# BAMresearch/fenics-constitutive

Hardware: AMD Instinct MI355X
Metric: quadrature-point stress updates/sec (Mpts/s) + % HBM roofline, 1/2/4/8 GPU (higher is better)
Workload: dtype f64; 1 GPU; von_mises_mixed: von_mises_3d FULL-3D, 100000000 pts/GPU device-resident, committed->trial evaluate, packed sparse history; points_per_gpu=100000000, points_total=100000000, parallelism=shard1

## Files before the change

fenics-constitutive_amd/_build.py:

```python

from __future__ import annotations

import os
import shutil
import subprocess
import sys

HERE = os.path.dirname(os.path.abspath(__file__))
CSRC = os.path.join(HERE, "csrc")
LIBDIR = os.path.join(HERE, "lib")
LIB = os.path.join(LIBDIR, "libfcamd.so")
SOURCES = ["fcamd_kernels.hip", "fcamd_aux_kernels.hip", "fcamd_capi.cpp", "fcamd_hostpath.cpp", "fcamd_hosttangent.cpp", "fcamd_multigpu.cpp", "fcamd_memory.cpp", "fcamd_multi.cpp"]
KERNEL_HEADERS = [os.path.join("kernels", h) for h in (
    "tile_io.h", "tangent_writers.h", "wrapped_io.h", "history_rows.h", "law_linear_elasticity.h", "law_sls.h",
    "law_von_mises.h", "law_comfe_mises.h", "law_drucker_prager.h", "law_lowdim.h", "stress_wrapped.h", "param_source.h")]
HEADERS = ["fcamd_internal.h", "fcamd_host.h", os.path.join("..", "..", "include", "fcamd.h"), os.path.join("..", "..", "include", "fcamd_multi.h"), *KERNEL_HEADERS]
ARCH = "gfx950"
FLAGS = ["-O3", "-std=c++17", "-fPIC", "-shared", "-pthread", "-ffp-contract=off", "-Wall", "-Wno-unused-function"]


HASHFILE = os.path.join(LIBDIR, "libfcamd.srchash")


def _source_hash() -> str:
    import hashlib

    h = hashlib.sha256(" ".join([ARCH, *FLAGS]).encode())
    for f in SOURCES + HEADERS:
        with open(os.path.join(CSRC, f), "rb") as fh:
            h.update(fh.read())
    return h.hexdigest()


KERNEL_SOURCES = ["fcamd_kernels.hip", "fcamd_internal.h", *KERNEL_HEADERS]
KERNEL_FLAGS = [f for f in FLAGS if f not in ("-pthread", "-fPIC", "-shared", "-Wall", "-Wno-unused-function")]
KERNEL_HASHFILE = os.path.join(LIBDIR, "libfcamd.kernelhash")


def _code_only(text: str) -> str:
    import re

    text = re.sub(r"/\*.*?\*/", " ", text, flags=re.S)
    text = re.sub(r"//[^\n]*", " ", text)
    return " ".join(text.split())


def kernel_hash(read=None) -> str:
    import hashlib

    if read is None:
        def read(f):
            with open(os.path.join(CSRC, f)) as fh:
                return fh.read()

    h = hashlib.sha256(" ".join([ARCH, *KERNEL_FLAGS]).encode())
    for f in KERNEL_SOURCES:
        h.update(f.encode() + b"\0" + _code_only(read(f)).encode() + b"\0")
    return h.hexdigest()


def built_kernel_hash():
    try:
        with open(KERNEL_HASHFILE) as fh:
            return fh.read().strip()
    except OSError:
        return None


def _stale() -> bool:
    if not (os.path.exists(LIB) and os.path.exists(HASHFILE)):
        return True
    with open(HASHFILE) as fh:
        return fh.read().strip() != _source_hash()


def build_library(force: bool = False, verbose: bool = False, keep_temps: bool = False) -> str:
    if not force and not _stale():
        return LIB
    hipcc = shutil.which("hipcc") or "/opt/rocm/bin/hipcc"
    if not os.path.exists(hipcc):
        raise RuntimeError("hipcc not found; cannot build libfcamd.so")
    os.makedirs(LIBDIR, exist_ok=True)
    tmp = f"{LIB}.{os.getpid()}.tmp"
    cmd = [hipcc, f"--offload-arch={ARCH}", *FLAGS]
    if keep_temps:
        bdir = os.path.join(CSRC, "build")
        os.makedirs(bdir, exist_ok=True)
        cmd += [f"-save-temps={'obj'}", "-Rpass-analysis=kernel-resource-usage"]
        tmp = os.path.join(bdir, "libfcamd.so")
    cmd += ["-o", tmp, *[os.path.join(CSRC, s) for s in SOURCES]]
    if verbose:
        print(" ".join(cmd), file=sys.stderr)
    r = subprocess.run(cmd, capture_output=True, text=True)
    if r.returncode != 0:
        raise RuntimeError(f"hipcc failed ({r.returncode}):\n{r.stdout}\n{r.stderr}")
    if keep_temps:
        shutil.copyfile(tmp, LIB + ".cp")
        os.replace(LIB + ".cp", LIB)
        sys.stderr.write(r.stderr)
# ... 14 lines not shown
```

fenics-constitutive_amd/csrc/fcamd_capi.cpp:

```cpp
#include <algorithm>
#include <chrono>
#include <cmath>
#include <cstdarg>
#include <cstdio>
#include <cstdlib>
#include <cstring>
#include <new>
#include <string>

#include "fcamd_host.h"

using namespace fcamd;

namespace fcamd {

thread_local std::string g_last_error;

int fail(int status, const char* fmt, ...) {
    char buf[512];
    va_list ap;
    va_start(ap, fmt);
    vsnprintf(buf, sizeof(buf), fmt, ap);
    va_end(ap);
    g_last_error = buf;
    return status;
}

}

namespace {

constexpr int kMaskedRowMaxVonMises = 20;
constexpr int kMaskedRowMaxRows7 = 16;

static_assert(fcamd::kCounterSlots == FCAMD_COUNTER_SLOTS, "public and internal counter layout differ");

constexpr double kFactorPy = 0x1.6a09e667f3bccp-1;
constexpr double kFactorRs = 0x1.6a09e667f3bcdp-1;

bool law_info(int id, LawInfo* li) {
    switch (id) {
        case FCAMD_LINEAR_ELASTICITY: *li = {2, 0, {}, false}; return true;
        case FCAMD_VON_MISES_3D: *li = {5, 2, {{"eps_n", 6}, {"alpha", 1}}, false}; return true;
        case FCAMD_SPRING_MAXWELL: *li = {4, 2, {{"strain_visco", 6}, {"strain", 6}}, true}; return true;
        case FCAMD_SPRING_KELVIN: *li = {4, 2, {{"strain_visco", 6}, {"strain", 6}}, true}; return true;
        case FCAMD_COMFE_LINEAR_ELASTICITY: *li = {2, 0, {}, false}; return true;
        case FCAMD_COMFE_MISES_PLASTICITY: *li = {4, 1, {{"history", 7}}, false}; return true;
        case FCAMD_COMFE_DRUCKER_PRAGER: *li = {5, 1, {{"history", 7}}, false}; return true;
        case FCAMD_COMFE_DRUCKER_PRAGER_HYPERBOLIC: *li = {6, 1, {{"history", 7}}, false}; return true;
        default: return false;
    }
}


void lame(double E, double nu, double* mu, double* lam) {
    *mu = E / (2.0 * (1.0 + nu));
    *lam = E * nu / ((1.0 + nu) * (1.0 - 2.0 * nu));
}

void elastic_tangent_full(double E, double nu, double D[36]) {
    double mu, lam;
    lame(E, nu, &mu, &lam);
    for (int i = 0; i < 36; ++i) D[i] = 0.0;
    for (int i = 0; i < 3; ++i)
        for (int j = 0; j < 3; ++j) D[6 * i + j] = (i == j) ? 2.0 * mu + lam : lam;
    for (int i = 3; i < 6; ++i) D[6 * i + i] = 2.0 * mu;
}

Dims dims_of(int constraint) {
    switch (constraint) {
        case FCAMD_UNIAXIAL_STRAIN:
        case FCAMD_UNIAXIAL_STRESS: return {1, 1, 1};
        case FCAMD_PLANE_STRAIN:
        case FCAMD_PLANE_STRESS: return {4, 4, 2};
        default: return {9, 6, 3};
    }
}

void elastic_tangent(double E, double nu, int constraint, double D[36]) {
    for (int i = 0; i < 36; ++i) D[i] = 0.0;
    double mu, lam;
    lame(E, nu, &mu, &lam);
    switch (constraint) {
        case FCAMD_FULL: elastic_tangent_full(E, nu, D); break;
        case FCAMD_PLANE_STRAIN:
            for (int i = 0; i < 3; ++i)
                for (int j = 0; j < 3; ++j) D[4 * i + j] = (i == j) ? 2.0 * mu + lam : lam;
            D[15] = 2.0 * mu;
            break;
        case FCAMD_PLANE_STRESS: {
            const double c = E / (1 - std::pow(nu, 2.0));
            const double M[16] = {1.0, nu, 0.0, 0.0, nu, 1.0, 0.0, 0.0, 0.0, 0.0, 0.0, 0.0, 0.0, 0.0, 0.0, (1.0 - nu)};
            for (int i = 0; i < 16; ++i) D[i] = c * M[i];
// ... 96 lines not shown
            sc.s[5] = mu0 / (tau * mu1);
            sc.s[6] = lam0 / (tau * 2 * mu1);
            const double w0 = 1 - mu0 / (tau * mu1 * factor);
            for (int i = 0; i < 36; ++i) {
                tb.a[i] = D0[i];
                tb.c[i] = w0 * D0[i];
            }
            break;
        }
        case FCAMD_COMFE_LINEAR_ELASTICITY: {
            const double mu = p[0], kappa = p[1];
            double soo[36], pvol[36], pdev[36];
            comfe_projections(soo, pvol, pdev);
            sc.s[0] = kFactorRs;
            for (int i = 0; i < 36; ++i) tb.a[i] = (2.0 * mu) * pdev[i] + (3.0 * kappa) * pvol[i];
            for (int i = 0; i < 6; ++i)
                for (int j = 0; j < 6; ++j) tb.c[6 * j + i] = tb.a[6 * i + j];
            break;
        }
        case FCAMD_COMFE_MISES_PLASTICITY: {
            const double mu = p[0], kappa = p[1], y_0 = p[2], h = p[3];
            double soo[36], pvol[36], pdev[36];
            comfe_projections(soo, pvol, pdev);
            sc.s[0] = kFactorRs;
            sc.s[1] = mu;
            sc.s[2] = kappa;
            sc.s[3] = y_0;
            sc.s[4] = h;
            sc.s[5] = 2. * mu;
            sc.s[6] = 3. * mu + h;
            sc.s[7] = std::sqrt(3. / 2.);
            sc.s[8] = 3. * mu;
            sc.s[9] = 1.0 / (1.0 + (h / (3.0 * mu)));
            for (int i = 0; i < 36; ++i) {
                tb.a[i] = kappa * soo[i];
                tb.b[i] = pdev[i];
            }
            break;
        }
        case FCAMD_COMFE_DRUCKER_PRAGER:
        case FCAMD_COMFE_DRUCKER_PRAGER_HYPERBOLIC: {
            const bool hyper = m->law == FCAMD_COMFE_DRUCKER_PRAGER_HYPERBOLIC;
            const double mu = p[0], kappa = p[1], a_ = p[2], b = p[3];
            const double d = hyper ? p[4] : 0.0, b_flow = hyper ? p[5] : p[4];
            double soo[36], pvol[36], pdev[36];
            comfe_projections(soo, pvol, pdev);
            sc.s[0] = kFactorRs;
            sc.s[1] = mu;
            sc.s[2] = kappa;
            sc.s[3] = a_;
            sc.s[4] = b;
            sc.s[5] = b_flow;
            sc.s[6] = d * d;
            sc.s[7] = 2.0 * mu;
            sc.s[8] = std::sqrt(2.0 / 3.0);
            sc.s[9] = 1.0 / (4.0 * mu);
            sc.s[10] = 1.0 / (9.0 * kappa);
            for (int i = 0; i < 36; ++i) {
                tb.a[i] = soo[i];
                tb.b[i] = pdev[i];
                tb.c[i] = (2.0 * mu) * pdev[i] + (3.0 * kappa) * pvol[i];
            }
            break;
        }
    }
}

void options_from_env(Options* o) {
    auto geti = [](const char* name, long long dflt) {
        const char* e = getenv(name);
        return (e && *e) ? atoll(e) : dflt;
    };
    o->masked_max = (int)geti("FCAMD_MASKED_MAX", -1);
    o->batch_kernel = geti("FCAMD_BATCH_KERNEL", 1) != 0;
    o->host_chunk = geti("FCAMD_HOST_CHUNK", 0);
    o->host_slots = (int)std::min<long long>(fcamd_context::kSlots, std::max<long long>(1, geti("FCAMD_HOST_SLOTS", fcamd_context::kSlots)));
    o->zero_copy = geti("FCAMD_ZERO_COPY", 1) != 0;
    o->zero_copy_grad = geti("FCAMD_ZERO_COPY_GRAD", 1) != 0;
    o->bounce_max = std::max<long long>(0, geti("FCAMD_BOUNCE_MAX", 256 << 10));
    o->host_tangent_threads = (int)geti("FCAMD_HOST_TANGENT_THREADS", -1);
    o->host_tangent_min_points = std::max<long long>(0, geti("FCAMD_HOST_TANGENT_MIN", 1 << 16));
    o->host_tangent_chunk = std::max<long long>(0, geti("FCAMD_HOST_TANGENT_CHUNK", 0));
    o->host_tangent_streams = (int)std::max<long long>(1, std::min<long long>(fcamd_context::kSlots, geti("FCAMD_HOST_TANGENT_STREAMS", 1)));
}

void constants_for(fcamd_model* m, double del_t) {
    if (m->const_valid && (m->const_del_t == del_t || !m->info.needs_del_t)) return;
    fill_constants(m, del_t, m->sc, m->tb);
    m->const_del_t = del_t;
    m->const_valid = true;
}

bool law_counts(int law) { return law == FCAMD_VON_MISES_3D || law >= FCAMD_COMFE_MISES_PLASTICITY; }

int timing_begin(fcamd_model* m) {
    fcamd_context* c = m->ctx;
    m->timed = c->timing;
    m->host_ms = -1.0f;
    if (m->timed) {
        if (law_counts(m->law)) HIP_TRY(hipMemsetAsync(m->d_counters, 0, kCounterBytes, c->stream));
        HIP_TRY(hipEventRecord(m->ev0, c->stream));
    }
    return FCAMD_OK;
}
int timing_end(fcamd_model* m) {
    if (m->timed) HIP_TRY(hipEventRecord(m->ev1, m->ctx->stream));
    return FCAMD_OK;
}

}

namespace fcamd {
static bool is_split(const fcamd_model* m, int flags) { return (flags & FCAMD_EVAL_SPLIT_HISTORY) != 0 && has_split_history(m->law); }

int validate_call(const fcamd_model* m, double del_t, int64_t n, const void* grad,
                  const void* stress_prev, const void* stress, const void* const* hist_prev,
                  const void* const* hist, int n_hist, int flags) {
    if (!m) return fail(FCAMD_ERR_BAD_ARG, "model handle is NULL");
    if (n < 0) return fail(FCAMD_ERR_SIZE, "negative number of quadrature points");
    if ((flags & FCAMD_EVAL_SPLIT_HISTORY) && !has_split_history(m->law))
        return fail(FCAMD_ERR_UNSUPPORTED, "FCAMD_EVAL_SPLIT_HISTORY exists for the laws with one [scalar, eps_p(6)] history row per point");
    if (n_hist < 0 || n_hist > FCAMD_MAX_HISTORY)
        return fail(FCAMD_ERR_SIZE, "n_hist = %d: 0 .. %d history fields exist", n_hist, FCAMD_MAX_HISTORY);
    if (m->info.n_hist == 0 && n_hist != 0)
        return fail(FCAMD_ERR_SIZE, "law has no history, got %d history fields", n_hist);
    if (m->info.n_hist > 0) {
        const int expected = (flags & FCAMD_EVAL_SPLIT_HISTORY) ? 2 : m->info.n_hist;
        if (!hist || !hist_prev || n_hist == 0)
            return fail(FCAMD_ERR_NULL_HISTORY, "history must not be None");
        if (n_hist != expected)
            return fail(FCAMD_ERR_SIZE, "law expects %d history fields, got %d", expected,
                        n_hist);
        for (int k = 0; k < n_hist; ++k)
            if (n > 0 && (!hist[k] || !hist_prev[k]))
                return fail(FCAMD_ERR_NULL_HISTORY, "history must not be None");
    }
    if (m->info.needs_del_t && !(del_t > 0.0))
        return fail(FCAMD_ERR_DEL_T, "Time step must be defined and positive.");
    if (n > 0 && (!grad || !stress || !stress_prev))
        return fail(FCAMD_ERR_BAD_ARG, "grad_del_u / stress pointer is NULL");
    return FCAMD_OK;
}

int check_protocol(const fcamd_model* m, int64_t n, const fcamd_eval_args* x) {
    if (x->flags & ~(FCAMD_EVAL_SPARSE_TANGENT | FCAMD_EVAL_SPLIT_HISTORY | FCAMD_EVAL_PACKED_HISTORY | FCAMD_EVAL_PARAM_FIELDS |
                     FCAMD_EVAL_GRAD_ON_DEVICE))
        return fail(FCAMD_ERR_UNSUPPORTED, "unknown FCAMD_EVAL_* flag in 0x%x (2, FCAMD_EVAL_DELTA_HISTORY of ABI 0.3, was removed in 0.4)", x->flags);
    if (x->history_mask && !has_sparse_history(m->law))
        return fail(FCAMD_ERR_UNSUPPORTED, "sparse trial history exists for the plasticity laws only");
    if ((x->flags & FCAMD_EVAL_PACKED_HISTORY) && n > 0) {
        const bool split = is_split(m, x->flags);
        if (m->law != FCAMD_VON_MISES_3D && !split)
            return fail(FCAMD_ERR_UNSUPPORTED, "FCAMD_EVAL_PACKED_HISTORY exists for VonMises3D and, with FCAMD_EVAL_SPLIT_HISTORY, for the "
                                               "comfe-rs plasticity laws");
        if (!x->history_mask || !x->packed_mask_prev || !x->packed_mask)
            return fail(FCAMD_ERR_BAD_ARG, "FCAMD_EVAL_PACKED_HISTORY needs history_mask, packed_mask_prev and packed_mask");
        if (x->parent_rows && m->law != FCAMD_VON_MISES_3D)
            return fail(FCAMD_ERR_UNSUPPORTED, "FCAMD_EVAL_PACKED_HISTORY with parent_rows: VonMises3D only");
        const int kd = split ? 1 : 0;
        if (x->history[kd] == x->history_prev[kd] || x->packed_mask == x->packed_mask_prev)
            return fail(FCAMD_ERR_BAD_ARG, "FCAMD_EVAL_PACKED_HISTORY needs trial plastic-strain and mask arrays of their own");
    }
    if (!aligned16(x->stress) || !aligned16(x->stress_prev))
        return fail(FCAMD_ERR_ALIGN, "device arrays must be 16-byte aligned");
    for (int k = 0; k < x->n_hist; ++k)
        if (!aligned16(x->history[k]) || !aligned16(x->history_prev[k]))
// ... 77 lines not shown

static bool host_mapped(fcamd_context* c, const void* p) {
    const char* q = static_cast<const char*>(p);
    if (c->bounce_dev && q >= c->bounce_dev && q < c->bounce_dev + c->bounce_bytes) return true;
    std::lock_guard<std::recursive_mutex> lock(c->host_mu);
    for (const auto& kv : c->registered)
        if (kv.second.dev && q >= kv.second.dev && q < kv.second.dev + kv.second.bytes) return true;
    return false;
}

static void fill_args(fcamd_model* m, double del_t, int64_t n, const Launch& l, EvalArgs& a) {
    a.grad = l.grad;
    a.stress_in = l.stress_prev;
    a.stress_out = l.stress;
    a.stress_out2 = l.stress2;
    a.tangent = l.tangent;
    const bool split = is_split(m, l.flags);
    const int nh = split ? 2 : m->info.n_hist;
    a.h0_in = nh > 0 ? l.hist_prev[0] : nullptr;
    a.h0_out = nh > 0 ? l.hist[0] : nullptr;
    a.h1_in = nh > 1 ? l.hist_prev[1] : nullptr;
    a.h1_out = nh > 1 ? l.hist[1] : nullptr;
    a.rows = l.rows;
    a.cache3d = nullptr;
    a.hmask = l.hmask;
    a.flags = split ? FCAMD_EVAL_SPLIT_HISTORY : 0;
    if (l.hmask) {
        if (l.tangent) a.flags |= l.flags & FCAMD_EVAL_SPARSE_TANGENT;
        if ((a.flags & FCAMD_EVAL_SPARSE_TANGENT) && host_mapped(m->ctx, l.tangent)) a.flags |= kFlagExactTangentRows;
        if ((m->law == FCAMD_VON_MISES_3D || (split && !l.rows)) && l.emask_prev && l.emask) a.flags |= l.flags & FCAMD_EVAL_PACKED_HISTORY;
    }
    if (m->ctx->twin_masks && m->law == FCAMD_VON_MISES_3D && !l.rows && (a.flags & FCAMD_EVAL_PACKED_HISTORY)) {
        a.flags |= 64;
        a.cache3d = reinterpret_cast<double*>(m->ctx->twin_masks);
    }
    if (l.tangent && (l.flags & kFlagTangentParamsHost)) a.flags = (a.flags & ~FCAMD_EVAL_SPARSE_TANGENT) | kFlagTangentParamsHost;
    a.emask_in = l.emask_prev;
    a.emask_out = l.emask;
    a.n = n;
    a.counters = l.counters ? l.counters : m->d_counters;
    const Options& o = m->ctx->opt;
    a.masked_max = o.masked_max >= 0 ? o.masked_max
                                     : ((m->law == FCAMD_VON_MISES_3D || split) ? kMaskedRowMaxVonMises : kMaskedRowMaxRows7);
    constants_for(m, del_t);
    a.sc = m->sc;
    a.tb = m->tb;
}

const double* const* fields_of(const fcamd_eval_args* x) {
    return (x->flags & FCAMD_EVAL_PARAM_FIELDS) ? reinterpret_cast<const double* const*>(x->stress_3d) : nullptr;
}

bool has_fields(const fcamd_model* m, const double* const* fields) {
    if (!fields) return false;
    for (int k = 0; k < m->info.n_params; ++k)
        if (fields[k]) return true;
    return false;
}

int check_fields(const fcamd_model* m, const double* const* fields) {
    if (!has_fields(m, fields)) return FCAMD_OK;
    if (!law_has_field_kernels(m->law) || m->constraint != FCAMD_FULL)
        return fail(FCAMD_ERR_UNSUPPORTED, "per-point parameter fields exist for LinearElasticityModel (FULL), LinearElasticity3D, VonMises3D "
                                           "and MisesPlasticityLinearHardening3D (model %d, constraint %d)", m->law, m->constraint);
    for (int k = 0; k < m->info.n_params; ++k)
        if (!aligned16(fields[k])) return fail(FCAMD_ERR_ALIGN, "parameter field %d must be 16-byte aligned", k);
    return FCAMD_OK;
}

static void field_args_for(const fcamd_model* m, const double* const* fields, int64_t p0, FieldArgs& f) {
    std::memset(&f, 0, sizeof(f));
    for (int k = 0; k < m->info.n_params; ++k) {
        f.f[k] = fields[k] ? fields[k] + p0 : nullptr;
        f.v[k] = m->params[k];
    }
}

static void field_tables(const fcamd_model* m, EvalArgs& a) {
    if (m->law != FCAMD_VON_MISES_3D && m->law != FCAMD_COMFE_MISES_PLASTICITY) return;
    for (int i = 0; i < 6; ++i)
        for (int j = 0; j < 6; ++j) a.tb.a[6 * i + j] = (i < 3 && j < 3) ? 1.0 : 0.0;
}

int enqueue(fcamd_model* m, double del_t, int64_t n, const Launch& l, hipStream_t stream, bool reset_counters) {
    EvalArgs a;
    fill_args(m, del_t, n, l, a);
    const bool per_point = has_fields(m, l.fields);
    if (per_point) {
        a.flags &= ~64;
        a.cache3d = nullptr;
        field_tables(m, a);
    }
    if ((reset_counters || l.counters) && law_counts(m->law)) HIP_TRY(hipMemsetAsync(a.counters, 0, kCounterBytes, stream));
    if (n == 0) return FCAMD_OK;
    const int grid = grid_for(m, n);
    (void)hipGetLastError();
    if (per_point) {
        FieldArgs f;
        field_args_for(m, l.fields, l.field_p0, f);
        HIP_TRY(launch_evaluate_fields(m->law, a, f, grid, stream));
        return FCAMD_OK;
    }
    HIP_TRY(launch_evaluate(m->law, m->dims.gdim, a, grid, stream));
    return FCAMD_OK;
}
}

namespace fcamd {
void constants_for_call(fcamd_model* m, double del_t) { constants_for(m, del_t); }

void sum_counters(const fcamd_model* m, fcamd_stats* out) {
    out->n_nonconverged = out->n_plastic = out->n_newton_iters = out->n_domain = 0;
    out->kernel_ms = -1.0;
    for (int s = 0; s < fcamd::kCounterSlots; ++s) {
        out->n_nonconverged += m->h_counters[4 * s + 0];
        out->n_plastic += m->h_counters[4 * s + 1];
        out->n_newton_iters += m->h_counters[4 * s + 2];
        out->n_domain += m->h_counters[4 * s + 3];
    }
}

int enqueue_counters_download(fcamd_model* m, hipStream_t stream) {
    HIP_TRY(hipMemcpyAsync(m->h_counters, m->d_counters, kCounterBytes, hipMemcpyDeviceToHost, stream));
    return FCAMD_OK;
}

int read_stats(fcamd_model* m, hipStream_t stream, fcamd_stats* out) {
    int st = enqueue_counters_download(m, stream);
    if (st != FCAMD_OK) return st;
    HIP_TRY(hipStreamSynchronize(stream));
    if (out) sum_counters(m, out);
    return FCAMD_OK;
}
}

static int evaluate_wrapped(fcamd_model* m, int wrapper_constraint, double del_t, int64_t n, const double* grad_lo, double* stress_lo,
                            double* tangent_lo, double* stress_3d, double* const* hist, int n_hist);

extern "C" {

int fcamd_version(void) { return FCAMD_VERSION_MAJOR * 1000 + FCAMD_VERSION_MINOR; }

int fcamd_device_count(int* count) {
    if (!count) return fail(FCAMD_ERR_BAD_ARG, "NULL argument");
    *count = 0;
    if (hipGetDeviceCount(count) != hipSuccess) {
        (void)hipGetLastError();
        *count = 0;
    }
    return FCAMD_OK;
}

const char* fcamd_last_error(void) { return g_last_error.c_str(); }

int fcamd_context_create(int device, void* stream, fcamd_context** out) {
    if (!out) return fail(FCAMD_ERR_BAD_ARG, "out is NULL");
    *out = nullptr;
    int count = 0;
    HIP_TRY(hipGetDeviceCount(&count));
    if (device < 0 || device >= count)
        return fail(FCAMD_ERR_BAD_ARG, "device %d out of range (%d devices)", device, count);
    HIP_TRY(hipSetDevice(device));
    fcamd_context* c = new (std::nothrow) fcamd_context();
    if (!c) return fail(FCAMD_ERR_BAD_ARG, "out of host memory");
    c->device = device;
    options_from_env(&c->opt);
    const int st = [&]() -> int {
        hipDeviceProp_t prop;
        HIP_TRY(hipGetDeviceProperties(&prop, device));
        c->num_cu = prop.multiProcessorCount > 0 ? prop.multiProcessorCount : 256;
        if (stream) {
            c->stream = static_cast<hipStream_t>(stream);
        } else {
            HIP_TRY(hipStreamCreateWithFlags(&c->stream, hipStreamNonBlocking));
            c->owns_stream = true;
        }
        return FCAMD_OK;
    }();
    if (st != FCAMD_OK) {
        delete c;
        return st;
    }
    *out = c;
    return FCAMD_OK;
}

static int context_trim(fcamd_context* c) {
    if (!c) return fail(FCAMD_ERR_BAD_ARG, "context is NULL");
    std::lock_guard<std::recursive_mutex> lock(c->host_mu);
    HIP_TRY(hipSetDevice(c->device));
    for (int i = 0; i < fcamd_context::kSlots; ++i)
        if (c->hstream[i]) HIP_TRY(hipStreamSynchronize(c->hstream[i]));
    free_host_staging(c);
    fcamd::host_tangent_release(c);
    return FCAMD_OK;
}

int fcamd_context_set_option(fcamd_context* c, const char* name, long long value) {
    if (!c || !name) return fail(FCAMD_ERR_BAD_ARG, "NULL argument");
    std::lock_guard<std::recursive_mutex> lock(c->host_mu);
    const std::string k(name);
    Options& o = c->opt;
    if (k == "masked_max") o.masked_max = (int)value;
    else if (k == "batch_kernel") o.batch_kernel = value != 0;
    else if (k == "host_chunk") o.host_chunk = value;
    else if (k == "host_slots") o.host_slots = (int)std::min<long long>(fcamd_context::kSlots, std::max<long long>(1, value));
    else if (k == "zero_copy") o.zero_copy = value != 0;
    else if (k == "zero_copy_grad") o.zero_copy_grad = value != 0;
    else if (k == "bounce_max") o.bounce_max = std::max<long long>(0, value);
    else if (k == "host_tangent_threads") o.host_tangent_threads = (int)std::max<long long>(-1, std::min<long long>(value, 256));
    else if (k == "host_tangent_min_points") o.host_tangent_min_points = std::max<long long>(0, value);
    else if (k == "host_tangent_chunk") o.host_tangent_chunk = std::max<long long>(0, (value / 64) * 64);
    else if (k == "host_tangent_streams") o.host_tangent_streams = (int)std::max<long long>(1, std::min<long long>(fcamd_context::kSlots, value));
    else if (k == "twin_masks") c->twin_masks = (unsigned long long)value;
    else if (k == "grid") c->grid_override = value > 0 ? (int)value : 0;
    else if (k == "timing") c->timing = value != 0;
    else if (k == "trim") return context_trim(c);
    else if (k == "peer_access") return fcamd::enable_peer_access(c, (int)value);
    else return fail(FCAMD_ERR_BAD_ARG, "unknown option '%s'", name);
    return FCAMD_OK;
}

int fcamd_context_get_option(fcamd_context* c, const char* name, long long* value) {
    if (!c || !name || !value) return fail(FCAMD_ERR_BAD_ARG, "NULL argument");
    const std::string k(name);
    const Options& o = c->opt;
    if (k == "masked_max") *value = o.masked_max;
    else if (k == "batch_kernel") *value = o.batch_kernel ? 1 : 0;
    else if (k == "host_chunk") *value = o.host_chunk;
    else if (k == "host_slots") *value = o.host_slots;
    else if (k == "zero_copy") *value = o.zero_copy;
    else if (k == "zero_copy_grad") *value = o.zero_copy_grad;
    else if (k == "bounce_max") *value = o.bounce_max;
    else if (k == "host_tangent_threads") *value = fcamd::host_tangent_threads(c);
    else if (k == "host_tangent_min_points") *value = o.host_tangent_min_points;
    else if (k == "host_tangent_chunk") *value = o.host_tangent_chunk;
    else if (k == "host_tangent_streams") *value = o.host_tangent_streams;
    else if (k == "last_host_tangent_cpu_us") *value = c->last_host_tangent_cpu_us;
    else if (k == "last_host_tangent_threads") *value = c->last_host_tangent_threads;
    else if (k == "grid") *value = c->grid_override;
    else if (k == "timing") *value = c->timing ? 1 : 0;
    else if (k == "last_host_mode") *value = c->last_host_mode;
    else return fail(FCAMD_ERR_BAD_ARG, "unknown option '%s'", name);
    return FCAMD_OK;
}

int fcamd_context_destroy(fcamd_context* c) {
    if (!c) return FCAMD_OK;
    (void)hipSetDevice(c->device);
    {
        std::lock_guard<std::recursive_mutex> lock(c->host_mu);
        release_registered_ranges(c);
    }
    free_host_staging(c);
    fcamd::host_tangent_release(c);
    for (int i = 0; i < fcamd_context::kSlots; ++i)
        if (c->hstream[i]) (void)hipStreamDestroy(c->hstream[i]);
    for (hipStream_t s : c->peer_streams)
        if (s) (void)hipStreamDestroy(s);
    for (hipEvent_t e : c->peer_events)
        if (e) (void)hipEventDestroy(e);
    for (auto& kv : c->ipc_open) (void)hipIpcCloseMemHandle(kv.second.base);
    for (auto& sl : c->batch_slots) {
        if (sl.host) (void)hipHostFree(sl.host);
        if (sl.dev) (void)hipFree(sl.dev);
        if (sl.uploaded) (void)hipEventDestroy(sl.uploaded);
    }
    if (c->owns_stream && c->stream) (void)hipStreamDestroy(c->stream);
    delete c;
    return FCAMD_OK;
}

int fcamd_context_set_stream(fcamd_context* c, void* stream) {
    if (!c) return fail(FCAMD_ERR_BAD_ARG, "context is NULL");
    if (c->owns_stream && c->stream) {
        (void)hipStreamDestroy(c->stream);
        c->owns_stream = false;
    }
    c->stream = static_cast<hipStream_t>(stream);
    return FCAMD_OK;
}

int fcamd_context_synchronize(fcamd_context* c) {
    if (!c) return fail(FCAMD_ERR_BAD_ARG, "context is NULL");
    HIP_TRY(hipStreamSynchronize(c->stream));
    return FCAMD_OK;
}

int fcamd_model_create(fcamd_context* c, int model_id, int constraint, const double* params,
                       int n_params, fcamd_model** out) {
    if (!out) return fail(FCAMD_ERR_BAD_ARG, "out is NULL");
    *out = nullptr;
    if (!c) return fail(FCAMD_ERR_BAD_ARG, "context is NULL");
    LawInfo li;
    if (!law_info(model_id, &li)) return fail(FCAMD_ERR_BAD_ARG, "unknown model id %d", model_id);
    if (constraint < FCAMD_UNIAXIAL_STRAIN || constraint > FCAMD_FULL)
        return fail(FCAMD_ERR_BAD_ARG, "unknown constraint %d", constraint);
    const bool all_constraints = model_id == FCAMD_LINEAR_ELASTICITY || model_id == FCAMD_SPRING_MAXWELL ||
                                 model_id == FCAMD_SPRING_KELVIN;
    if (constraint != FCAMD_FULL && !all_constraints)
        return fail(FCAMD_ERR_UNSUPPORTED, "model %d is implemented for StressStrainConstraint.FULL only (got %d)",
                    model_id, constraint);
    if (!params || n_params != li.n_params)
        return fail(FCAMD_ERR_BAD_ARG, "model %d expects %d parameters, got %d", model_id,
                    li.n_params, n_params);
    HIP_TRY(hipSetDevice(c->device));
    fcamd_model* m = new (std::nothrow) fcamd_model();
    if (!m) return fail(FCAMD_ERR_BAD_ARG, "out of host memory");
    m->ctx = c;
    m->law = model_id;
    m->constraint = constraint;
    m->dims = dims_of(constraint);
    if (all_constraints)
        for (int k = 0; k < li.n_hist; ++k) li.hist[k].dim = m->dims.sd;
    m->info = li;
    for (int i = 0; i < n_params; ++i) m->params[i] = params[i];
    hipError_t e = hipMalloc(reinterpret_cast<void**>(&m->d_counters), kCounterBytes);
    if (e == hipSuccess)
        e = hipHostMalloc(reinterpret_cast<void**>(&m->h_counters), kCounterBytes,
                          hipHostMallocDefault);
// ... 305 lines not shown
```

fenics-constitutive_amd/csrc/fcamd_host.h:

```cpp
#pragma once
#include "../../include/fcamd.h"
#include "../../include/fcamd_multi.h"

#include <cstdint>
#include <map>
#include <mutex>
#include <string>
#include <vector>

#include "fcamd_internal.h"

namespace fcamd {

int fail(int status, const char* fmt, ...) __attribute__((format(printf, 2, 3)));

#define HIP_TRY(expr)                                                                  \
    do {                                                                               \
        hipError_t e_ = (expr);                                                        \
        if (e_ != hipSuccess) {                                                        \
            (void)hipGetLastError();  \
            return ::fcamd::fail(FCAMD_ERR_HIP, "%s failed: %s (%s:%d)", #expr, hipGetErrorString(e_), \
                                 __FILE__, __LINE__);                                  \
        }                                                                              \
    } while (0)

struct HistField {
    const char* name;
    int dim;
};

struct LawInfo {
    int n_params;
    int n_hist;
    HistField hist[FCAMD_MAX_HISTORY];
    bool needs_del_t;
};

struct Dims {
    int gd2, sd, gdim;
};

struct Options {
    bool batch_kernel = true;
    int masked_max = -1;
    long long host_chunk = 0;
    int host_slots = 4;
    int zero_copy = 1;
    int zero_copy_grad = 1;
    long long bounce_max = 256 << 10;
    int host_tangent_threads = -1;
    long long host_tangent_min_points = 1 << 16;
    long long host_tangent_chunk = 0;
    int host_tangent_streams = 1;
};

struct HostTangentJob {
    enum Kind { CONST = 0, MISES = 1, MISES_COMFE = 2, DRUCKER_PRAGER = 3 } kind;
    int prm;
    int td;
    const double* table_a;
    const double* table_b;
    const double* table_c;
    double* tangent;
    double elastic_row[36];
};
class ExpandPool;

}

struct fcamd_context {
    int device = 0;
    int num_cu = 256;
    hipStream_t stream = nullptr;
    bool owns_stream = false;
    int grid_override = 0;
    bool timing = false;
    fcamd::Options opt;
    static constexpr int kSlots = 4;
    hipStream_t hstream[kSlots] = {nullptr, nullptr, nullptr, nullptr};
    double* dchunk[kSlots] = {nullptr, nullptr, nullptr, nullptr};
    size_t dchunk_points = 0;
    int64_t chunk_points = 0;
    struct Pinned {
        size_t bytes;
        char* dev;
        bool borrowed = false;
        char* lock_base = nullptr;
    };
    std::map<char*, Pinned> registered;
    std::recursive_mutex host_mu;
    int last_host_mode = 0;
    unsigned long long twin_masks = 0;
    char* bounce = nullptr;
    char* bounce_dev = nullptr;
    size_t bounce_bytes = 0;
    std::vector<hipStream_t> peer_streams;
    std::vector<hipEvent_t> peer_events;
    struct IpcMapping {
        void* base;
        int refs;
    };
    std::map<std::string, IpcMapping> ipc_open;
    static constexpr int kBatchMax = 32;
    static constexpr int kBatchSlots = 16;
    struct BatchSlot {
        fcamd::BatchEntry* host = nullptr;
        fcamd::BatchEntry* dev = nullptr;
        size_t bytes = 0;
        uint64_t hash = 0;
        hipEvent_t uploaded = nullptr;
        hipStream_t stream = nullptr;
    };
    BatchSlot batch_slots[kBatchSlots];
    unsigned batch_next = 0;
    std::vector<fcamd::BatchEntry> batch_build;
    fcamd::ExpandPool* pool = nullptr;
    char* tparams = nullptr;
    char* tparams_dev = nullptr;
    size_t tparams_bytes = 0;
    static constexpr int kTangentSlots = 16;
    hipEvent_t tp_event[kTangentSlots] = {};
    long long last_host_tangent_cpu_us = 0;
    int last_host_tangent_threads = 0;
};

struct fcamd_model {
    fcamd_context* ctx = nullptr;
    int law = 0;
    int constraint = FCAMD_FULL;
    fcamd::Dims dims{9, 6, 3};
    fcamd::LawInfo info{};
    double params[8] = {0};
    unsigned long long* d_counters = nullptr;
    unsigned long long* h_counters = nullptr;
    hipEvent_t ev0 = nullptr, ev1 = nullptr;
    bool timed = false;
    float host_ms = -1.0f;
    int grid_auto = 0;
    bool const_valid = false;
    double const_del_t = 0.0;
    fcamd::Scalars sc;
    fcamd::Tables tb;
};

namespace fcamd {

constexpr size_t kCounterBytes = (size_t)kCounterSlots * 4 * sizeof(unsigned long long);

inline bool has_sparse_history(int law) { return law == FCAMD_VON_MISES_3D || law >= FCAMD_COMFE_MISES_PLASTICITY; }

inline bool has_split_history(int law) { return law >= FCAMD_COMFE_MISES_PLASTICITY; }

inline bool aligned16(const void* p) { return (reinterpret_cast<uintptr_t>(p) & 15u) == 0; }

int validate_call(const fcamd_model* m, double del_t, int64_t n, const void* grad, const void* stress_prev,
                  const void* stress, const void* const* hist_prev, const void* const* hist, int n_hist, int flags = 0);

int enable_peer_access(fcamd_context* c, int peer_device);
size_t ipc_safe_alloc_size(size_t bytes);

struct Launch {
    const double *grad = nullptr, *stress_prev = nullptr;
    double *stress = nullptr, *stress2 = nullptr;
    double* tangent = nullptr;
    const double* hist_prev[FCAMD_MAX_HISTORY] = {};
    double* hist[FCAMD_MAX_HISTORY] = {};
    const int* rows = nullptr;
    unsigned long long* hmask = nullptr;
    const unsigned long long* emask_prev = nullptr;
    unsigned long long *emask = nullptr, *counters = nullptr;
    const double* const* fields = nullptr;
    int64_t field_p0 = 0;
    int flags = 0;
};
// ... 48 lines not shown
```

Baseline: 12960 Mpts/s.

## Add specialized resident von Mises kernel with row-pair sparse tangent writes

Adds a dedicated grid-stride kernel for full-3D von Mises with sparse tangent and packed history. It picks between eager and deferred packed-history loads based on the plastic mask and writes sparse tangent rows in pairs using 36 lanes of 16-byte stores. Any tail of fewer than 64 points goes to the generic kernel. The aim is less wasted memory traffic and fewer tangent store passes in the device-resident case, at the cost of a second code path and an extra launch for tails.

```diff
diff --git a/fenics-constitutive_amd/_build.py b/fenics-constitutive_amd/_build.py
--- a/fenics-constitutive_amd/_build.py
+++ b/fenics-constitutive_amd/_build.py
@@ -10,11 +10,14 @@
 CSRC = os.path.join(HERE, "csrc")
 LIBDIR = os.path.join(HERE, "lib")
 LIB = os.path.join(LIBDIR, "libfcamd.so")
-SOURCES = ["fcamd_kernels.hip", "fcamd_aux_kernels.hip", "fcamd_capi.cpp", "fcamd_hostpath.cpp", "fcamd_hosttangent.cpp", "fcamd_multigpu.cpp", "fcamd_memory.cpp", "fcamd_multi.cpp"]
+SOURCES = ["fcamd_kernels.hip", "fcamd_aux_kernels.hip", "fcamd_capi.cpp", "fcamd_hostpath.cpp", "fcamd_hosttangent.cpp", "fcamd_multigpu.cpp", "fcamd_memory.cpp", "fcamd_multi.cpp",
+           os.path.join("resident", "fcamd_resident_kernels.hip")]
 KERNEL_HEADERS = [os.path.join("kernels", h) for h in (
     "tile_io.h", "tangent_writers.h", "wrapped_io.h", "history_rows.h", "law_linear_elasticity.h", "law_sls.h",
     "law_von_mises.h", "law_comfe_mises.h", "law_drucker_prager.h", "law_lowdim.h", "stress_wrapped.h", "param_source.h")]
-HEADERS = ["fcamd_internal.h", "fcamd_host.h", os.path.join("..", "..", "include", "fcamd.h"), os.path.join("..", "..", "include", "fcamd_multi.h"), *KERNEL_HEADERS]
+RESIDENT_HEADERS = [os.path.join("resident", h) for h in ("fcamd_resident.h", "tangent_row_pairs.h")]
+HEADERS = ["fcamd_internal.h", "fcamd_host.h", os.path.join("..", "..", "include", "fcamd.h"), os.path.join("..", "..", "include", "fcamd_multi.h"), *KERNEL_HEADERS,
+           *RESIDENT_HEADERS]
 ARCH = "gfx950"
 FLAGS = ["-O3", "-std=c++17", "-fPIC", "-shared", "-pthread", "-ffp-contract=off", "-Wall", "-Wno-unused-function"]
 
diff --git a/fenics-constitutive_amd/csrc/fcamd_capi.cpp b/fenics-constitutive_amd/csrc/fcamd_capi.cpp
--- a/fenics-constitutive_amd/csrc/fcamd_capi.cpp
+++ b/fenics-constitutive_amd/csrc/fcamd_capi.cpp
@@ -9,6 +9,7 @@
 #include <string>
 
 #include "fcamd_host.h"
+#include "resident/fcamd_resident.h"
 
 using namespace fcamd;
 
@@ -271,6 +272,7 @@
     o->host_tangent_min_points = std::max<long long>(0, geti("FCAMD_HOST_TANGENT_MIN", 1 << 16));
     o->host_tangent_chunk = std::max<long long>(0, geti("FCAMD_HOST_TANGENT_CHUNK", 0));
     o->host_tangent_streams = (int)std::max<long long>(1, std::min<long long>(fcamd_context::kSlots, geti("FCAMD_HOST_TANGENT_STREAMS", 1)));
+    o->resident_kernel = (int)std::max<long long>(0, std::min<long long>(2, geti("FCAMD_RESIDENT_KERNEL", 1)));
 }
 
 void constants_for(fcamd_model* m, double del_t) {
@@ -514,6 +516,31 @@
         for (int j = 0; j < 6; ++j) a.tb.a[6 * i + j] = (i < 3 && j < 3) ? 1.0 : 0.0;
 }
 
+static bool resident_kernel_applies(const fcamd_model* m, const Launch& l, const EvalArgs& a, int grid) {
+    const int mode = m->ctx->opt.resident_kernel;
+    if (mode <= 0 || m->law != FCAMD_VON_MISES_3D || m->constraint != FCAMD_FULL || l.rows) return false;
+    if (a.flags != (FCAMD_EVAL_SPARSE_TANGENT | FCAMD_EVAL_PACKED_HISTORY) || !a.hmask || !a.tangent) return false;
+    const int64_t tiles = a.n / 64;
+    return tiles >= 1 && (mode >= 2 || tiles >= (int64_t)grid * 4);
+}
+
+static void tail_args(EvalArgs& a) {
+    const int64_t p0 = (a.n / 64) * 64;
+    a.grad += 9 * p0;
+    a.stress_in += 6 * p0;
+    a.stress_out += 6 * p0;
+    if (a.stress_out2) a.stress_out2 += 6 * p0;
+    a.tangent += 36 * p0;
+    a.h0_in += 6 * p0;
+    a.h0_out += 6 * p0;
+    a.h1_in += p0;
+    a.h1_out += p0;
+    a.hmask += p0 / 64;
+    a.emask_in += p0 / 64;
+    a.emask_out += p0 / 64;
+    a.n -= p0;
+}
+
 int enqueue(fcamd_model* m, double del_t, int64_t n, const Launch& l, hipStream_t stream, bool reset_counters) {
     EvalArgs a;
     fill_args(m, del_t, n, l, a);
@@ -524,6 +551,7 @@
         field_tables(m, a);
     }
     if ((reset_counters || l.counters) && law_counts(m->law)) HIP_TRY(hipMemsetAsync(a.counters, 0, kCounterBytes, stream));
+    m->ctx->last_resident_kernel = 0;
     if (n == 0) return FCAMD_OK;
     const int grid = grid_for(m, n);
     (void)hipGetLastError();
@@ -531,6 +559,15 @@
         FieldArgs f;
         field_args_for(m, l.fields, l.field_p0, f);
         HIP_TRY(launch_evaluate_fields(m->law, a, f, grid, stream));
+        return FCAMD_OK;
+    }
+    if (resident_kernel_applies(m, l, a, grid)) {
+        m->ctx->last_resident_kernel = 1;
+        HIP_TRY(launch_evaluate_resident_vm(a, grid, stream));
+        if (n % 64 != 0) {
+            tail_args(a);
+            HIP_TRY(launch_evaluate(m->law, m->dims.gdim, a, 1, stream));
+        }
         return FCAMD_OK;
     }
     HIP_TRY(launch_evaluate(m->law, m->dims.gdim, a, grid, stream));
@@ -644,6 +681,7 @@
     else if (k == "host_tangent_min_points") o.host_tangent_min_points = std::max<long long>(0, value);
     else if (k == "host_tangent_chunk") o.host_tangent_chunk = std::max<long long>(0, (value / 64) * 64);
     else if (k == "host_tangent_streams") o.host_tangent_streams = (int)std::max<long long>(1, std::min<long long>(fcamd_context::kSlots, value));
+    else if (k == "resident_kernel") o.resident_kernel = (int)std::max<long long>(0, std::min<long long>(2, value));
     else if (k == "twin_masks") c->twin_masks = (unsigned long long)value;
     else if (k == "grid") c->grid_override = value > 0 ? (int)value : 0;
     else if (k == "timing") c->timing = value != 0;
@@ -668,6 +706,8 @@
     else if (k == "host_tangent_min_points") *value = o.host_tangent_min_points;
     else if (k == "host_tangent_chunk") *value = o.host_tangent_chunk;
     else if (k == "host_tangent_streams") *value = o.host_tangent_streams;
+    else if (k == "resident_kernel") *value = o.resident_kernel;
+    else if (k == "last_resident_kernel") *value = c->last_resident_kernel;
     else if (k == "last_host_tangent_cpu_us") *value = c->last_host_tangent_cpu_us;
     else if (k == "last_host_tangent_threads") *value = c->last_host_tangent_threads;
     else if (k == "grid") *value = c->grid_override;
diff --git a/fenics-constitutive_amd/csrc/fcamd_host.h b/fenics-constitutive_amd/csrc/fcamd_host.h
--- a/fenics-constitutive_amd/csrc/fcamd_host.h
+++ b/fenics-constitutive_amd/csrc/fcamd_host.h
@@ -52,6 +52,7 @@
     long long host_tangent_min_points = 1 << 16;
     long long host_tangent_chunk = 0;
     int host_tangent_streams = 1;
+    int resident_kernel = 1;
 };
 
 struct HostTangentJob {
@@ -90,6 +91,7 @@
     std::map<char*, Pinned> registered;
     std::recursive_mutex host_mu;
     int last_host_mode = 0;
+    int last_resident_kernel = 0;
     unsigned long long twin_masks = 0;
     char* bounce = nullptr;
     char* bounce_dev = nullptr;
diff --git a/fenics-constitutive_amd/csrc/resident/fcamd_resident.h b/fenics-constitutive_amd/csrc/resident/fcamd_resident.h
--- /dev/null
+++ b/fenics-constitutive_amd/csrc/resident/fcamd_resident.h
@@ -0,0 +1,8 @@
+#pragma once
+#include "../fcamd_internal.h"
+
+namespace fcamd {
+
+hipError_t launch_evaluate_resident_vm(const EvalArgs& args, int grid, hipStream_t stream);
+
+}
diff --git a/fenics-constitutive_amd/csrc/resident/fcamd_resident_kernels.hip b/fenics-constitutive_amd/csrc/resident/fcamd_resident_kernels.hip
--- /dev/null
+++ b/fenics-constitutive_amd/csrc/resident/fcamd_resident_kernels.hip
@@ -0,0 +1,124 @@
+#include "fcamd_resident.h"
+
+#include "../kernels/tile_io.h"
+#include "../kernels/tangent_writers.h"
+#include "../kernels/history_rows.h"
+#include "../kernels/param_source.h"
+#include "../kernels/law_von_mises.h"
+#include "tangent_row_pairs.h"
+
+namespace fcamd {
+
+__device__ __forceinline__ void tile_resident_von_mises(ArgsRef a, const StressBases& sb, const Tables* T, double* region, long long p0,
+                                                        int lane, WaveStats& st) {
+    constexpr bool NT = true;
+    const unsigned long long m_old = a.hmask[p0 >> 6];
+    PackedRows<true, NT> pk;
+    pk.ever_in = a.emask_in[p0 >> 6];
+    const unsigned long long ever_trial = a.emask_out[p0 >> 6];
+    Chunks<9> cg;
+    StressRows<false, true, NT> sr;
+    tile_load<9, true, NT>(cg, a.grad + p0 * 9, kWave * 9, lane);
+    sr.load(a, sb, p0, kWave, lane, nullptr);
+    const double alpha_n = a.h1_in[p0 + lane];
+    const VMUniform prm{a.sc};
+    const int run_rows = (int)__popcll(pk.ever_in);
+    const bool same_layout = ever_trial == pk.ever_in && run_rows >= kPackedRowsMinRun;
+    const bool early = m_old != 0ull && !(same_layout && kPackedRowsDiv * (int)__popcll(m_old) <= run_rows);
+    if (early) pk.load(a.h0_in, p0, lane);
+    double g[9], s[6], e[6];
+    transpose_in<9>(cg, region, lane, g);
+    sr.get(region, lane, s);
+    mandel_strain(g, a.sc.s[0], e);
+
+    VMTrial tr;
+    vm_trial(prm, e, s, alpha_n, tr);
+    const bool plastic = tr.phitr > 0.0;
+    const unsigned long long mask = __ballot(plastic);
+    const unsigned long long need_mask = mask | m_old;
+    const bool touched = need_mask != 0ull;
+    if (!early && touched) {
+        if (same_layout && (mask & ~pk.ever_in) == 0ull && kPackedRowsDiv * (int)__popcll(need_mask) <= run_rows)
+            pk.load_rows(a.h0_in, p0, lane, need_mask, region);
+        else
+            pk.load(a.h0_in, p0, lane);
+    }
+
+    VMReturn rm;
+    if (mask != 0ull) {
+        if (plastic) vm_return(prm, tr, alpha_n, rm, st);
+        st.plastic += (lane == 0) ? (unsigned long long)__popcll(mask) : 0ull;
+    }
+
+    double ep[6] = {0.0, 0.0, 0.0, 0.0, 0.0, 0.0};
+    if (touched) pk.gather(region, lane, ep);
+
+    vm_stress(prm, tr, rm, s);
+    sr.put(sb, region, lane, s, p0, kWave, nullptr);
+
+    if (touched) {
+#pragma unroll
+        for (int i = 0; i < 6; ++i) ep[i] = plastic ? ep[i] + rm.gamma * rm.N[i] : ep[i];
+        pk.scatter(a, a.h0_out, p0, lane, mask, region, ep);
+        a.h1_out[p0 + lane] = alpha_n + a.sc.s[3] * rm.gamma;
+    }
+    if (lane == 0 && mask != m_old) a.hmask[p0 >> 6] = mask;
+
+    if (touched) {
+        double B, C;
+        vm_tangent_coefficients(prm, rm, B, C);
+        publish_tangent_params(region, lane, B, C, rm.N);
+        wave_sync();
+        double* tile = sb.tan + p0 * 36;
+        const unsigned long long need = uniform64(need_mask);
+        if (need == ~0ull)
+            tangent_mises_passes<false, NT, false, false>(region, T->a, T->b, tile, lane, need, false, std::make_integer_sequence<int, 18>{});
+        else if (tangent_pairs_needed(need) <= kPairPassesMax)
+            tangent_mises_row_pairs<NT>(region, T->a, T->b, tile, lane, need);
+        else
+            tangent_mises_passes<false, NT, true, false>(region, T->a, T->b, tile, lane, need, false, std::make_integer_sequence<int, 18>{});
+        wave_sync();
+    }
+}
+
+__global__ void __launch_bounds__(kBlock, 4) evaluate_resident_vm_kernel(const EvalArgs) {
+    ArgsRef a = kernel_args();
+    __shared__ __attribute__((aligned(16))) Tables T;
+    __shared__ __attribute__((aligned(16))) double scratch[kWavesPerBlock][kRegionDoubles];
+    {
+        const double FCAMD_CONSTANT* src = (const double FCAMD_CONSTANT*)&a.tb;
+        double* dst = reinterpret_cast<double*>(&T);
+        for (int i = threadIdx.x; i < 108; i += blockDim.x) dst[i] = src[i];
+        __syncthreads();
+    }
+    int lane = threadIdx.x & (kWave - 1);
+    const int wave = __builtin_amdgcn_readfirstlane((int)(threadIdx.x / kWave));
+    double* region = scratch[wave];
+    const long long nfull = a.n / kWave;
+    const long long wstride = (long long)gridDim.x * kWavesPerBlock;
+    const StressBases sb{a.stress_in, a.stress_out, a.tangent, a.stress_out2};
+    WaveStats st;
+    for (long long tile = (long long)blockIdx.x * kWavesPerBlock + wave; tile < nfull; tile += wstride) {
+        asm volatile("" : "+v"(lane));
+        lane &= kWave - 1;
+        tile_resident_von_mises(a, sb, &T, region, tile * kWave, lane, st);
+    }
+    const unsigned long long nc = wave_sum(st.nonconv);
+    const unsigned long long np = wave_sum(st.plastic);
+    const unsigned long long ni = wave_sum(st.iters);
+    if (lane == 0) {
+        unsigned long long* c = a.counters + 4 * ((int)blockIdx.x & (kCounterSlots - 1));
+        if (nc) atomicAdd(c + 0, nc);
+        if (np) atomicAdd(c + 1, np);
+        if (ni) atomicAdd(c + 2, ni);
+    }
+}
+
+hipError_t launch_evaluate_resident_vm(const EvalArgs& args, int grid, hipStream_t stream) {
+    constexpr int want = kFlagSparseTangent | kFlagPackedHistory;
+    if (args.flags != want || !args.hmask || !args.emask_in || !args.emask_out || !args.tangent || args.rows) return hipErrorInvalidValue;
+    if (args.n >= kWave) hipLaunchKernelGGL(evaluate_resident_vm_kernel, dim3(grid), dim3(kBlock), 0, stream, args);
+    return hipGetLastError();
+}
+
+}
diff --git a/fenics-constitutive_amd/csrc/resident/tangent_row_pairs.h b/fenics-constitutive_amd/csrc/resident/tangent_row_pairs.h
--- /dev/null
+++ b/fenics-constitutive_amd/csrc/resident/tangent_row_pairs.h
@@ -0,0 +1,76 @@
+#pragma once
+#include <utility>
+
+#include "../kernels/tile_io.h"
+#include "../kernels/tangent_writers.h"
+
+namespace fcamd {
+
+constexpr int kPairLanes = 36;
+constexpr int kPairPasses = 32;
+
+constexpr int kPairPassesMax = 20;
+__device__ __forceinline__ int tangent_pairs_needed(unsigned long long need) {
+    return (int)__popcll((need | (need >> 1)) & 0x5555555555555555ull);
+}
+
+struct PairLane {
+    const double* bc;
+    const double* ni;
+    const double* nj;
+    d2 a, b;
+    unsigned w_lo, w_hi;
+    char* dst;
+};
+
+__device__ __forceinline__ PairLane pair_lane(const double* tp, const double* ta, const double* tb, double* tile, int lane,
+                                              unsigned long long need) {
+    PairLane c;
+    const int second = lane >= 18 ? 1 : 0;
+    const int r = min(lane - 18 * second, 17);
+    const int i = (int)(__umul24((unsigned)r, 11u) >> 5);
+    const int jj = r - __mul24(3, i);
+    const double* t = tp + 10 * second;
+    c.bc = t;
+    c.ni = t + 2 + i;
+    c.nj = t + 2 + 2 * jj;
+    c.a = *reinterpret_cast<const d2*>(ta + 2 * r);
+    c.b = *reinterpret_cast<const d2*>(tb + 2 * r);
+    const unsigned long long up = need >> 1;
+    const unsigned long long w = lane < 16 ? need : (lane < 20 ? (need | up) : (lane < kPairLanes ? up : 0ull));
+    c.w_lo = (unsigned)w;
+    c.w_hi = (unsigned)(w >> 32);
+    c.dst = reinterpret_cast<char*>(tile) + (unsigned)lane * 16u;
+    return c;
+}
+
+template <bool NT, int M>
+__device__ __forceinline__ void tangent_pair_pass(const PairLane& c, unsigned long long need) {
+    if (((need >> (2 * M)) & 3ull) == 0ull) return;
+    asm volatile("");
+    constexpr unsigned bit = 1u << ((2 * M) & 31);
+    const unsigned word = 2 * M < 32 ? c.w_lo : c.w_hi;
+    if ((word & bit) != 0u) {
+        const d2 bc = *reinterpret_cast<const d2*>(c.bc + 20 * M);
+        const double ni = c.ni[20 * M];
+        const d2 nj = *reinterpret_cast<const d2*>(c.nj + 20 * M);
+        d2 v;
+        v.x = (c.a.x + bc.x * c.b.x) + bc.y * (ni * nj.x);
+        v.y = (c.a.y + bc.x * c.b.y) + bc.y * (ni * nj.y);
+        store_tangent16<NT>(reinterpret_cast<double*>(c.dst + M * (kPairLanes * 16)), v);
+    }
+}
+
+template <bool NT, int... M>
+__device__ __forceinline__ void tangent_pair_passes(const PairLane& c, unsigned long long need, std::integer_sequence<int, M...>) {
+    (tangent_pair_pass<NT, M>(c, need), ...);
+}
+
+template <bool NT>
+__device__ __forceinline__ void tangent_mises_row_pairs(const double* tp, const double* ta, const double* tb, double* tile, int lane,
+                                                        unsigned long long need) {
+    const PairLane c = pair_lane(tp, ta, tb, tile, lane, need);
+    tangent_pair_passes<NT>(c, need, std::make_integer_sequence<int, kPairPasses>{});
+}
+
+}
```

Measured after the change: 13050 Mpts/s (median of 4 runs). No clear change (+0.6%).
